# eloialonso/diamond

Measured on NVIDIA H100. Metric: imagined frames/sec (64x64, 3 denoise steps), higher is better.
Workload: dtype fp16 tensor-core operands (split-fp16 on the residual-stream 1x1/conv_in layers), fp32 accumulate, fp32 activations

## Files before the change

diamond_b200/csrc/api.cu:

```cuda
#include <cstdlib>
#include <memory>
#include <mutex>
#include <map>
#include <cuda_runtime.h>

#include <cmath>
#include <cstdarg>
#include <cstdio>
#include <cstring>
#include <functional>
#include <string>
#include <vector>

#include "../../include/diamond_b200.h"
#include "aux_kernels.cuh"
#include "conv_tc.cuh"
#include "wgrad_tc.cuh"
#include "bwd_kernels.cuh"
#include "optim_kernels.cuh"

using namespace dmd;

static thread_local std::string g_err;
static thread_local long long g_launches = 0;
// ... 116 lines not shown
    const int cs[2] = {d->C0, d->C1};
    const int nsrc = d->C1 ? 2 : 1;
    int n = 0;
    for (int rep = 0; rep < (d->precise ? 3 : 1); ++rep)
      for (int k = 0; k < nsrc; ++k) { p->seg_base[n] = (rep == 1) ? lo[k] : hi[k]; p->seg_slabs[n] = cs[k] / 16; ++n; }
    p->Cin = (d->C0 + d->C1) * (d->precise ? 3 : 1);
    p->Cextra = 0;
    if (d->wpk_x) {
      DMD_CHECK(d->xsrc0 && d->xsrc0_lo && d->xC0 > 0 && d->xC0 % 16 == 0 && d->xC1 % 16 == 0 && d->xC0 + d->xC1 <= kMaxCin, "conv: bad fused projection operands");
      DMD_CHECK((d->xC1 == 0) == (d->xsrc1 == nullptr) && (d->xC1 == 0) == (d->xsrc1_lo == nullptr), "conv: fused projection src1 mismatch");
      const uint8_t* xh[2] = {(const uint8_t*)d->xsrc0, (const uint8_t*)d->xsrc1};
      const uint8_t* xl[2] = {(const uint8_t*)d->xsrc0_lo, (const uint8_t*)d->xsrc1_lo};
      const int xc[2] = {d->xC0, d->xC1};
      for (int rep = 0; rep < 2; ++rep)
        for (int k = 0; k < (d->xC1 ? 2 : 1); ++k) {
          DMD_CHECK(n < kMaxSegs, "conv: too many operand segments");
          p->seg_base[n] = (rep == 1) ? xl[k] : xh[k]; p->seg_slabs[n] = xc[k] / 16; ++n;
        }
      p->Cextra = 3 * (d->xC0 + d->xC1);
      p->xslabs = 2 * (d->xC0 + d->xC1) / 16;
      p->wpk_extra = reinterpret_cast<const __half*>(d->wpk_x);
      p->bias_extra = d->bias_x;
    }
    p->nseg = n;
  }
  p->B = d->B; p->H = d->H; p->W = d->W; p->taps = d->taps; p->stride = d->stride;
  if (d->stride == 2) DMD_CHECK(p->H % 2 == 0 && p->W % 2 == 0, "conv: stride 2 needs even H,W");
  p->wpk = reinterpret_cast<const __half*>(d->wpk); p->bias = d->bias; p->Cout = d->Cout; p->CoutPad = d->CoutPad;
  p->resid = d->residual; p->out = d->out; p->ostats = d->out_stats; p->ogs = d->out_gs > 0 ? d->out_gs : d->Cout;
  const Plc g = plc_geometry(d->B, d->H, d->W);
  p->PW = g.PW; p->PH = g.PH; p->Q = g.Q; p->G = g.G; p->plane_bytes = (unsigned long long)g.Qalloc * 16;
  DMD_CHECK((long long)g.Q * (g.PW > g.PH ? g.PW : g.PH) < (1ll << 32), "conv: problem too large for 32-bit position math");
  p->trs = d->wpk_layout == 1 ? 1 : 0;
  if (p->trs) DMD_CHECK(d->taps == 9 && !d->precise && 3 * d->CoutPad <= 256, "conv: row-stacked weights need a 3x3, non-split conv with CoutPad <= 80");
  const int halo = d->taps == 9 ? g.PW + 1 : 0;
  p->P = kTileM + 2 * halo; p->Palloc = p->P | 1;
  if (d->out_stats) {
    const int L4 = d->Cout / 4;
    DMD_CHECK(g.PH * g.PW >= 64, "conv: image too small for the statistics epilogue (a tile may touch at most %d images)", kStatSlots);
    DMD_CHECK(d->Cout % 4 == 0 && (L4 == 4 || L4 == 8 || L4 == 16 || L4 == 32), "conv: out_stats needs Cout in {16,32,64,128} (got %d)", d->Cout);
    DMD_CHECK(d->out_gs == 16 || d->out_gs == 32 || d->out_gs == 64 || d->out_gs == 128, "conv: out_gs must be 16/32/64/128");
    DMD_CHECK(d->Cout % d->out_gs == 0 && d->Cout / d->out_gs <= kMaxOutGroups, "conv: bad output groups");
  }
  p->dPW.init(g.PW); p->dPH.init(g.PH);
  p->num_tiles = (g.Q + kTileM - 1) / kTileM;
  const int kslabs = p->Cin / 16 + p->xslabs;
  const uint32_t w_bytes = conv_weight_bytes(p->taps, p->Cin, p->Cextra, p->CoutPad);
  const ConvSmemLayout L0 = conv_smem_layout(w_bytes, p->Palloc, 0);
  const long long budget = 227ll * 1024 - (long long)L0.total;
  int stages = budget > 0 ? (int)(budget / (long long)L0.slab_bytes) : 0;
  if (stages > 4 * kslabs) stages = 4 * kslabs;
  if (stages > kMaxStages) stages = kMaxStages;
  DMD_CHECK(stages >= 2, "conv: shared memory too small for W=%d Cin=%d CoutPad=%d", p->W, p->Cin, p->CoutPad);
  p->stages = stages;
  *smem = conv_smem_layout(w_bytes, p->Palloc, stages).total;
  *acc_cols = d->CoutPad <= 16 ? 16 : (d->CoutPad <= 32 ? 32 : (d->CoutPad <= 64 ? 64 : 128));
  return 0;
}

struct DevState { int num_sms = 0; void* zeros = nullptr; };
static thread_local int g_num_sms = 0;
static thread_local const uint8_t* g_zeros = nullptr;
static int init_kernels() {
  static std::mutex mu;
  static std::map<int, DevState> states;
  int dev = 0;
  DMD_CUDA(cudaGetDevice(&dev));
  std::lock_guard<std::mutex> lk(mu);
  auto it = states.find(dev);
  if (it == states.end()) {
    DevState st;
    DMD_CUDA(cudaDeviceGetAttribute(&st.num_sms, cudaDevAttrMultiProcessorCount, dev));
    DMD_CUDA(cudaFuncSetAttribute(conv_tc_kernel<16, 9>, cudaFuncAttributeMaxDynamicSharedMemorySize, 227 * 1024));
    DMD_CUDA(cudaFuncSetAttribute(conv_tc_kernel<32, 9>, cudaFuncAttributeMaxDynamicSharedMemorySize, 227 * 1024));
    DMD_CUDA(cudaFuncSetAttribute(conv_tc_kernel<64, 9>, cudaFuncAttributeMaxDynamicSharedMemorySize, 227 * 1024));
    DMD_CUDA(cudaFuncSetAttribute(conv_tc_kernel<128, 9>, cudaFuncAttributeMaxDynamicSharedMemorySize, 227 * 1024));
    DMD_CUDA(cudaFuncSetAttribute(conv_tc_kernel<16, 1>, cudaFuncAttributeMaxDynamicSharedMemorySize, 227 * 1024));
    DMD_CUDA(cudaFuncSetAttribute(conv_tc_kernel<32, 1>, cudaFuncAttributeMaxDynamicSharedMemorySize, 227 * 1024));
    DMD_CUDA(cudaFuncSetAttribute(conv_tc_kernel<64, 1>, cudaFuncAttributeMaxDynamicSharedMemorySize, 227 * 1024));
    DMD_CUDA(cudaFuncSetAttribute(conv_tc_kernel<128, 1>, cudaFuncAttributeMaxDynamicSharedMemorySize, 227 * 1024));
    DMD_CUDA(cudaFuncSetAttribute(wgrad_tc_kernel<16>, cudaFuncAttributeMaxDynamicSharedMemorySize, 227 * 1024));
    DMD_CUDA(cudaFuncSetAttribute(wgrad_tc_kernel<32>, cudaFuncAttributeMaxDynamicSharedMemorySize, 227 * 1024));
    DMD_CUDA(cudaFuncSetAttribute(wgrad_tc_kernel<64>, cudaFuncAttributeMaxDynamicSharedMemorySize, 227 * 1024));
    DMD_CUDA(cudaFuncSetAttribute(attn_cluster_kernel<64>, cudaFuncAttributeMaxDynamicSharedMemorySize, 128 * 1024));
    DMD_CUDA(cudaFuncSetAttribute(attn_cluster_kernel<32>, cudaFuncAttributeMaxDynamicSharedMemorySize, 128 * 1024));
    DMD_CUDA(cudaFuncSetAttribute(attn_kernel<64>, cudaFuncAttributeMaxDynamicSharedMemorySize, 128 * 1024));
    DMD_CUDA(cudaFuncSetAttribute(attn_kernel<32>, cudaFuncAttributeMaxDynamicSharedMemorySize, 128 * 1024));
    DMD_CUDA(cudaFuncSetAttribute(attn_bwd_kernel<64>, cudaFuncAttributeMaxDynamicSharedMemorySize, 200 * 1024));
    DMD_CUDA(cudaFuncSetAttribute(attn_bwd_kernel<32>, cudaFuncAttributeMaxDynamicSharedMemorySize, 200 * 1024));
    DMD_CUDA(cudaFuncSetAttribute(linear_kernel<4>, cudaFuncAttributeMaxDynamicSharedMemorySize, 64 * 1024));
    DMD_CUDA(cudaFuncSetAttribute(linear_kernel<2>, cudaFuncAttributeMaxDynamicSharedMemorySize, 64 * 1024));
    DMD_CUDA(cudaFuncSetAttribute(linear_kernel<1>, cudaFuncAttributeMaxDynamicSharedMemorySize, 64 * 1024));
    DMD_CUDA(cudaMalloc(&st.zeros, 4096));
    DMD_CUDA(cudaMemset(st.zeros, 0, 4096));
    it = states.emplace(dev, st).first;
  }
  g_num_sms = it->second.num_sms;
  g_zeros = (const uint8_t*)it->second.zeros;
  return 0;
}

template <typename Kernel, typename Params>
static int launch_pdl(Kernel kernel, dim3 grid, dim3 block, size_t smem, cudaStream_t st, const Params& p) {
  cudaLaunchConfig_t cfg;
  memset(&cfg, 0, sizeof(cfg));
  cfg.gridDim = grid; cfg.blockDim = block; cfg.dynamicSmemBytes = smem; cfg.stream = st;
  cudaLaunchAttribute attr[1];
  attr[0].id = cudaLaunchAttributeProgrammaticStreamSerialization;
  attr[0].val.programmaticStreamSerializationAllowed = 1;
  cfg.attrs = attr; cfg.numAttrs = tune_int("DMD_NO_PDL", 0) ? 0 : 1;
  DMD_CUDA(cudaLaunchKernelEx(&cfg, kernel, p));
  DMD_LAUNCH_OK();
  return 0;
}

template <int kCols>
static int conv_launch_t(const ConvParams& p0, size_t smem, cudaStream_t st) {
  if (init_kernels()) return 1;
  const int grid = p0.num_tiles < g_num_sms ? p0.num_tiles : g_num_sms;
  ConvParams p = p0;
  p.ktrace = kt_slot(p.taps == 9 ? "conv3x3" : "conv1x1", p.num_tiles, (p.Cin + p.Cextra) * 1000 + p.W);
  if (p.taps == 9) return launch_pdl(conv_tc_kernel<kCols, 9>, dim3(grid), dim3(kConvThreads), smem, st, p);
  return launch_pdl(conv_tc_kernel<kCols, 1>, dim3(grid), dim3(kConvThreads), smem, st, p);
}

static int prep_fill(const dmd_prep_desc* d, PrepParams* p, int* nsrc) {
  DMD_CHECK(d->src0 && d->dst0, "prep: null src0/dst0");
  DMD_CHECK(d->C0 % 8 == 0 && d->C1 % 8 == 0 && d->C0 > 0 && d->C0 <= kMaxCin && d->C1 <= kMaxCin, "prep: channels must be multiples of 8 (C0=%d C1=%d)", d->C0, d->C1);
  DMD_CHECK((d->C1 == 0) == (d->src1 == nullptr) && (d->C1 == 0) == (d->dst1 == nullptr), "prep: src1/dst1/C1 mismatch");
  DMD_CHECK(d->mode >= 0 && d->mode <= 2, "prep: bad mode");
  for (int c : {d->C0, d->C1 ? d->C1 : 16}) {
    const int cp = round_up(c, 16);
    DMD_CHECK(cp == 16 || cp == 32 || cp == 64 || cp == 128, "prep: a source must have <= 16/32/64/128 channels after padding (got %d)", c);
  }
  memset(p, 0, sizeof(*p));
  p->s[0].src = d->src0; p->s[0].C = d->C0; p->s[0].Cpad = round_up(d->C0, 16); p->s[0].stats = d->stats0; p->s[0].gs = d->gs0 > 0 ? d->gs0 : 8;
  p->s[0].c_offset = 0; p->s[0].dst = (uint8_t*)d->dst0; p->s[0].dst_raw = (uint8_t*)d->dst_raw0;
  p->s[0].dst_lo = (uint8_t*)d->dst_lo0; p->s[0].dst_raw_lo = (uint8_t*)d->dst_raw_lo0;
  p->s[1].dst_lo = (uint8_t*)d->dst_lo1; p->s[1].dst_raw_lo = (uint8_t*)d->dst_raw_lo1;
  DMD_CHECK(!(d->dst_raw_lo0 && !d->dst_raw0) && !(d->dst_raw_lo1 && !d->dst_raw1), "prep: raw low part needs the raw operand too");
  p->s[1].src = d->src1; p->s[1].C = d->C1; p->s[1].Cpad = round_up(d->C1 > 0 ? d->C1 : 16, 16); p->s[1].stats = d->stats1; p->s[1].gs = d->gs1 > 0 ? d->gs1 : 8;
  p->s[1].c_offset = d->C0; p->s[1].dst = (uint8_t*)d->dst1; p->s[1].dst_raw = (uint8_t*)d->dst_raw1;
  if (d->mode) {
    DMD_CHECK(d->stats0 && d->gs0 > 0 && d->C0 % d->gs0 == 0, "prep: norm mode needs stats0/gs0");
    if (d->C1) DMD_CHECK(d->stats1 && d->gs1 > 0 && d->C1 % d->gs1 == 0, "prep: norm mode needs stats1/gs1");
    if (d->mode == 1) DMD_CHECK(d->film != nullptr, "prep: AdaGroupNorm needs film");
    if (d->mode == 2) DMD_CHECK(d->gamma && d->beta, "prep: GroupNorm needs gamma/beta");
    DMD_CHECK(d->upsample == 0, "prep: norm + upsample unsupported");
  }
  p->B = d->B; p->Hs = d->Hs; p->Ws = d->Ws; p->ups = d->upsample;
  DMD_CHECK(d->upsample >= 0 && d->upsample <= 2, "prep: upsample must be 0, 1 (nearest 2x) or 2 (zero insertion)");
  DMD_CHECK(d->upsample != 2 || (d->mode == 0 && !d->silu && d->C1 == 0 && !d->dst_raw0 && !d->dst_lo0), "prep: zero insertion is a raw single-source operand");
  p->H = d->upsample ? 2 * d->Hs : d->Hs; p->W = d->upsample ? 2 * d->Ws : d->Ws;
  p->mode = d->mode; p->act = d->silu ? 1 : 0;
  p->film = d->film; p->film_stride = d->film_stride; p->film_off = d->film_off; p->film_ctot = d->C0 + d->C1;
  p->gamma = d->gamma; p->beta = d->beta; p->eps = d->eps;
// ... 2549 lines not shown
```

diamond_b200/csrc/conv_tc.cuh:

```cuda
#pragma once
#include "ptx.cuh"

namespace dmd {

constexpr int kConvThreads = 384;
constexpr int kConvConsumerWarps = 8;
constexpr int kTileM = 128;
constexpr int kMaxCin = 128;
constexpr int kMaxSegs = 8;
constexpr int kMaxStages = 24;
constexpr int kStatSlots = 3;
constexpr int kMaxOutGroups = 4;

struct FastDiv {
  uint32_t d, m;
  __host__ void init(uint32_t dd) {
    d = dd;
    m = (uint32_t)((0x100000000ull / dd) + 1);
  }
  __device__ __forceinline__ uint32_t div(uint32_t n) const { return d == 1 ? n : __umulhi(n, m); }
};

struct Plc {
  int PW, PH, Q, G, Qalloc;
};
__host__ __device__ inline Plc plc_geometry(int B, int H, int W) {
  Plc g;
  g.PW = W + 1; g.PH = H + 1; g.Q = B * g.PH * g.PW; g.G = g.PW + 1;
  g.Qalloc = g.G + ((g.Q + kTileM - 1) / kTileM) * kTileM + kTileM + g.PW + 1;
  return g;
}

struct ConvParams {
  const uint8_t* seg_base[kMaxSegs];
  int seg_slabs[kMaxSegs];
  int nseg;
  int Cin;
  int Cextra;
  const __half* wpk_extra;
  const float* bias_extra;
  int xslabs;
  int B, H, W;
  int taps;
  int stride;
  const __half* wpk;
  const float* bias;
  int Cout, CoutPad;
  const float* resid;
  float* out;
  double* ostats;
  int ogs;
  int PW, PH, Q, G;
  unsigned long long plane_bytes;
  int P, Palloc;
  int num_tiles, stages;
  int trs;
  FastDiv dPW, dPH;
  long long* ktrace;
};

struct ConvSmemLayout {
  uint32_t bias_off, w_off, a_off, slab_bytes, total;
};

__host__ __device__ inline uint32_t conv_weight_bytes(int taps, int Cin, int Cextra, int CoutPad) {
  return (((uint32_t)taps * Cin * CoutPad * 2 + 127u) & ~127u) + (uint32_t)Cextra * CoutPad * 2;
}
__host__ __device__ inline ConvSmemLayout conv_smem_layout(uint32_t w_bytes, int Palloc, int stages) {
  ConvSmemLayout L;
  L.bias_off = 512;
  L.w_off = L.bias_off + 128 * 4;
  L.a_off = (L.w_off + w_bytes + 127u) & ~127u;
  L.slab_bytes = 2u * Palloc * 16;
  L.total = L.a_off + (uint32_t)stages * L.slab_bytes + 16;
  return L;
}

template <int N>
struct RegEpilogue {
  int lane, r0, G;
  float s[kStatSlots][kMaxOutGroups], ss[kStatSlots][kMaxOutGroups];
  int n_cur;

  __device__ __forceinline__ void init(const ConvParams& p, int row0, int lane_) {
    lane = lane_;
    r0 = row0;
    G = p.ostats ? p.Cout / p.ogs : 1;
#pragma unroll
    for (int k = 0; k < kStatSlots; ++k)
#pragma unroll
      for (int g = 0; g < kMaxOutGroups; ++g) s[k][g] = ss[k][g] = 0.f;
    n_cur = -1;
  }

  __device__ __forceinline__ void flush_stats(const ConvParams& p, int img0, int nslots) {
#pragma unroll
    for (int k = 0; k < kStatSlots; ++k) {
#pragma unroll
      for (int g = 0; g < kMaxOutGroups; ++g) {
        if (k < nslots && g < G) {
          float a = s[k][g], b = ss[k][g];
#pragma unroll
          for (int m = 16; m > 0; m >>= 1) {
            a += __shfl_xor_sync(0xffffffffu, a, m);
            b += __shfl_xor_sync(0xffffffffu, b, m);
          }
          if (lane == 0 && img0 + k < p.B && (a != 0.f || b != 0.f)) {
            double* dst = p.ostats + ((size_t)(img0 + k) * G + g) * 2;
            atomicAdd(dst, (double)a);
            atomicAdd(dst + 1, (double)b);
          }
        }
        s[k][g] = ss[k][g] = 0.f;
      }
    }
  }

  template <int kLgs>
  __device__ __forceinline__ void tile(const ConvParams& p, const float* sbias, const float (&acc)[N / 2], int q0) {
    constexpr bool kStats = kLgs > 0;
    constexpr int kGroups = (N / 8) >> kLgs > 0 ? ((N / 8) >> kLgs < kMaxOutGroups ? (N / 8) >> kLgs : kMaxOutGroups) : 1;
    const int n_lo = (int)p.dPH.div(p.dPW.div((uint32_t)q0));
    const int q_last = min(q0 + kTileM, p.Q) - 1;
    const bool single_image = (int)p.dPH.div(p.dPW.div((uint32_t)q_last)) == n_lo;
    if (kStats && n_cur >= 0 && (!single_image || n_lo != n_cur)) { flush_stats(p, n_cur, 1); n_cur = -1; }
    const int c0 = 2 * (lane & 3);
    const bool vec = (p.Cout & 1) == 0;
#pragma unroll
    for (int h = 0; h < 2; ++h) {
      const int q = q0 + r0 + 8 * h;
      int opix = -1, slot = 0;
      if (q < p.Q) {
        const uint32_t R = p.dPW.div((uint32_t)q);
        const int x = q - (int)R * p.PW;
        const int n = (int)p.dPH.div(R);
        const int y = (int)R - n * p.PH;
        bool valid = (x < p.W) && (y < p.H);
        int yo = y, xo = x, Ho = p.H, Wo = p.W;
        if (p.stride == 2) {
          valid = valid && ((x & 1) == 0) && ((y & 1) == 0);
          yo = y >> 1; xo = x >> 1; Ho = p.H >> 1; Wo = p.W >> 1;
        }
        if (valid) { opix = (n * Ho + yo) * Wo + xo; slot = n - n_lo; }
      }
      if (opix < 0) continue;
      float* op = p.out + (size_t)opix * p.Cout;
      const float* rp = p.resid != nullptr ? p.resid + (size_t)opix * p.Cout : nullptr;
      float gs[kMaxOutGroups], gss[kMaxOutGroups];
#pragma unroll
      for (int g = 0; g < kMaxOutGroups; ++g) gs[g] = gss[g] = 0.f;
      constexpr int kBatch = N / 8 < 8 ? N / 8 : 8;
#pragma unroll
      for (int jb = 0; jb < N / 8; jb += kBatch) {
        float2 bv[kBatch], rv[kBatch];
#pragma unroll
        for (int u = 0; u < kBatch; ++u) {
          const int col = 8 * (jb + u) + c0;
          bv[u] = rv[u] = make_float2(0.f, 0.f);
          if (col < p.Cout) {
            bv[u] = make_float2(sbias[col], sbias[col + 1]);
            if (rp) {
              if (vec) rv[u] = __ldg(reinterpret_cast<const float2*>(rp + col));
              else {
                rv[u].x = __ldg(rp + col);
                if (col + 1 < p.Cout) rv[u].y = __ldg(rp + col + 1);
              }
            }
          }
        }
#pragma unroll
        for (int u = 0; u < kBatch; ++u) {
          const int j = jb + u;
          const int col = 8 * j + c0;
          if (col < p.Cout) {
            float2 o = make_float2(acc[4 * j + 2 * h] + bv[u].x, acc[4 * j + 2 * h + 1] + bv[u].y);
            if (vec) {
              if (rp) { o.x += rv[u].x; o.y += rv[u].y; }
              *reinterpret_cast<float2*>(op + col) = o;
            } else {
              if (rp) o.x += rv[u].x;
              op[col] = o.x;
              if (col + 1 < p.Cout) { if (rp) o.y += rv[u].y; op[col + 1] = o.y; } else o.y = 0.f;
            }
            if (kStats) {
              gs[j >> kLgs] += o.x + o.y;
              gss[j >> kLgs] += fmaf(o.x, o.x, o.y * o.y);
            }
          }
        }
      }
      if (kStats) {
        if (single_image) {
#pragma unroll
          for (int g = 0; g < kGroups; ++g) { s[0][g] += gs[g]; ss[0][g] += gss[g]; }
        } else {
#pragma unroll
          for (int k = 0; k < kStatSlots; ++k)
#pragma unroll
            for (int g = 0; g < kGroups; ++g) { s[k][g] += (slot == k) ? gs[g] : 0.f; ss[k][g] += (slot == k) ? gss[g] : 0.f; }
        }
      }
    }
    if (kStats) {
      if (single_image) n_cur = n_lo;
      else { flush_stats(p, n_lo, kStatSlots); n_cur = -1; }
    }
  }

  __device__ __forceinline__ void finish(const ConvParams& p) {
    if (p.ostats != nullptr && n_cur >= 0) flush_stats(p, n_cur, 1);
  }
};

template <int N, int kTaps>
__global__ void __launch_bounds__(kConvThreads, 1) conv_tc_kernel(const ConvParams p) {
  extern __shared__ __align__(128) uint8_t smem[];
  uint64_t* wbar = reinterpret_cast<uint64_t*>(smem);
  uint64_t* full = wbar + 1;
  uint64_t* empty = full + kMaxStages;
  const ConvSmemLayout L = conv_smem_layout(conv_weight_bytes(p.taps, p.Cin, p.Cextra, p.CoutPad), p.Palloc, p.stages);
  float* sbias = reinterpret_cast<float*>(smem + L.bias_off);
  uint8_t* sW = smem + L.w_off;
  uint8_t* sA = smem + L.a_off;

  const int tid = threadIdx.x;
  const int warp = tid >> 5, lane = tid & 31;
  const int halo = (kTaps == 9) ? (p.PW + 1) : 0;
  const int S = p.stages;
  const int main_slabs = p.Cin >> 4;
  const int kslabs = main_slabs + p.xslabs;
  const uint32_t w_main_bytes = ((uint32_t)p.taps * p.Cin * p.CoutPad * 2 + 127u) & ~127u;
  const int tiles_lo = p.num_tiles / (int)gridDim.x, tiles_rem = p.num_tiles % (int)gridDim.x;
  const int tile_begin = (int)blockIdx.x * tiles_lo + min((int)blockIdx.x, tiles_rem);
  const int my_tiles = tiles_lo + ((int)blockIdx.x < tiles_rem ? 1 : 0);

  pdl_launch_dependents();
  if (tid == 0) {
    mbar_init(wbar, 1);
    for (int s = 0; s < S; ++s) { mbar_init(full + s, 1); mbar_init(empty + s, kConvConsumerWarps); }
    fence_mbar_init();
    const uint32_t tap_bytes = (uint32_t)p.Cin * p.CoutPad * 2;
    const uint32_t extra_bytes = (uint32_t)p.Cextra * p.CoutPad * 2;
    mbar_expect_tx(wbar, tap_bytes * p.taps + extra_bytes);
    for (int t = 0; t < p.taps; ++t)
      bulk_g2s(sW + (size_t)t * tap_bytes, reinterpret_cast<const uint8_t*>(p.wpk) + (size_t)t * tap_bytes, tap_bytes, wbar);
    if (extra_bytes) bulk_g2s(sW + w_main_bytes, p.wpk_extra, extra_bytes, wbar);
  }
  for (int i = tid; i < 128; i += blockDim.x)
    sbias[i] = ((p.bias != nullptr && i < p.Cout) ? __ldg(p.bias + i) : 0.f) + ((p.bias_extra != nullptr && i < p.Cout) ? __ldg(p.bias_extra + i) : 0.f);
  __syncthreads();
  pdl_wait();
  if (blockIdx.x == 0 && tid == 128) ktrace_stamp(p.ktrace);

  if (warp < 2) {
    const uint32_t pid = (uint32_t)warp;
    const uint32_t chunk_bytes = (uint32_t)p.P * 16;
    uint32_t stage = 0, phase = 0, nslab = 0;
    for (int it = 0; it < my_tiles; ++it) {
      const size_t pos0 = (size_t)((tile_begin + it) * kTileM - halo + p.G) * 16;
      int seg = 0, seg_ks = 0;
      for (int ks = 0; ks < kslabs; ++ks, ++nslab) {
        if ((nslab & 1u) == pid) {
          mbar_wait(empty + stage, phase ^ 1u);
          if (elect_one_sync()) {
            uint8_t* slab = sA + (size_t)stage * L.slab_bytes;
            const bool xs = ks >= main_slabs;
            const uint32_t bytes = xs ? (uint32_t)kTileM * 16 : chunk_bytes;
            mbar_expect_tx(full + stage, 2 * bytes);
            const uint8_t* plane = p.seg_base[seg] + (size_t)(2 * seg_ks) * p.plane_bytes + pos0 + (xs ? (size_t)halo * 16 : 0);
            bulk_g2s(slab, plane, bytes, full + stage);
            bulk_g2s(slab + (size_t)p.Palloc * 16, plane + p.plane_bytes, bytes, full + stage);
          }
          __syncwarp();
        }
        if (++seg_ks == p.seg_slabs[seg]) { seg_ks = 0; ++seg; }
        if (++stage == (uint32_t)S) { stage = 0; phase ^= 1u; }
      }
    }
  } else if (warp >= 4) {
    const int m0 = ((warp >> 2) - 1) * 64;
    RegEpilogue<N> epi;
    epi.init(p, m0 + 16 * (warp & 3) + (lane >> 2), lane);
    const int lgs = p.ostats ? 31 - __clz(p.ogs >> 3) : 0;
    if (my_tiles > 0) mbar_wait(wbar, 0);
    const uint64_t hi = gmma_desc_hi(128);
    const uint32_t a_lbo = (uint32_t)p.Palloc * 16;
    const uint32_t b_lbo = (uint32_t)(p.trs ? 3 * p.CoutPad : p.CoutPad) * 16;
    const uint32_t x_lbo = (uint32_t)p.CoutPad * 16;
    const uint32_t a_lo0 = (((smem_u32(sA) + (uint32_t)m0 * 16) >> 4) & 0x3FFFu) | (((a_lbo >> 4) & 0x3FFFu) << 16);
    const uint32_t b_lo0 = ((smem_u32(sW) >> 4) & 0x3FFFu) | (((b_lbo >> 4) & 0x3FFFu) << 16);
    const uint32_t b_x0 = (((smem_u32(sW) + w_main_bytes) >> 4) & 0x3FFFu) | (((x_lbo >> 4) & 0x3FFFu) << 16);
    const uint32_t slab16 = L.slab_bytes >> 4;
    const uint32_t kstep16 = (2u * b_lbo) >> 4;
    const uint32_t xstep16 = (2u * x_lbo) >> 4;
    uint32_t shift[kTaps], b_tap[kTaps];
#pragma unroll
    for (int t = 0; t < kTaps; ++t) {
      shift[t] = (uint32_t)(halo + (kTaps == 9 ? (t / 3 - 1) * p.PW + (t % 3 - 1) : 0));
      b_tap[t] = p.trs ? ((uint32_t)(t / 3) * p.Cin * 3u * p.CoutPad * 2 + (uint32_t)(t % 3) * p.CoutPad * 16) >> 4
                       : ((uint32_t)t * p.Cin * p.CoutPad * 2) >> 4;
    }
    const int ng = p.xslabs >> 1;
    float acc[N / 2];
    uint32_t stage = 0, phase = 0, prev = 0;
    int done = 0;
    auto slab = [&](auto issue) {
      mbar_wait(full + stage, phase);
      wgmma_fence();
      issue(a_lo0 + stage * slab16);
      wgmma_commit();
      wgmma_wait<1>();
      if (done > 0 && lane == 0) mbar_arrive(empty + prev);
      prev = stage;
      ++done;
      if (++stage == (uint32_t)S) { stage = 0; phase ^= 1u; }
    };
    for (int it = 0; it < my_tiles; ++it) {
#pragma unroll
      for (int i = 0; i < N / 2; ++i) acc[i] = 0.f;
      done = 0;
      for (int ks = 0; ks < main_slabs; ++ks) {
        const uint32_t b_lo = b_lo0 + (uint32_t)ks * kstep16;
        slab([&](uint32_t a_lo) {
#pragma unroll
          for (int t = 0; t < kTaps; ++t) Wgmma<N>::template mma<0, 0>(acc, hi | (a_lo + shift[t]), hi | (b_lo + b_tap[t]), 1u);
        });
      }
      for (int g = 0; g < ng; ++g)
        slab([&](uint32_t a_lo) {
          Wgmma<N>::template mma<0, 0>(acc, hi | a_lo, hi | (b_x0 + (uint32_t)g * xstep16), 1u);
          Wgmma<N>::template mma<0, 0>(acc, hi | a_lo, hi | (b_x0 + (uint32_t)(2 * ng + g) * xstep16), 1u);
        });
      for (int g = 0; g < ng; ++g)
        slab([&](uint32_t a_lo) { Wgmma<N>::template mma<0, 0>(acc, hi | a_lo, hi | (b_x0 + (uint32_t)(ng + g) * xstep16), 1u); });
      wgmma_wait<0>();
      wgmma_fence_operands(acc);
      if (done > 0 && lane == 0) mbar_arrive(empty + prev);
      const int q0 = (tile_begin + it) * kTileM;
      if (lgs == 0) epi.template tile<0>(p, sbias, acc, q0);
      else if (lgs == 1 || N == 16) epi.template tile<1>(p, sbias, acc, q0);
      else if (lgs == 2 || N == 32) epi.template tile<2>(p, sbias, acc, q0);
      else if (lgs == 3 || N == 64) epi.template tile<3>(p, sbias, acc, q0);
      else epi.template tile<4>(p, sbias, acc, q0);
    }
    epi.finish(p);
  }
}

struct PrepSrc {
  const float* src;
  int C;
  int Cpad;
  const double* stats;
  int gs;
  int c_offset;
  uint8_t* dst;
  uint8_t* dst_lo;
  uint8_t* dst_raw;
  uint8_t* dst_raw_lo;
};
struct PrepParams {
  PrepSrc s[2];
  int B, Hs, Ws, ups, H, W;
  int mode;
  int act;
  const float* film;
  int film_stride, film_off, film_ctot;
  const float* gamma;
  const float* beta;
  float eps;
  int PW, PH, Q, G, Qalloc;
  unsigned long long plane_bytes;
  int pos_per_block;
  FastDiv dPW, dPH;
  long long* ktrace;
};

constexpr int kPrepThreads = 256;
// ... 300 lines not shown
```

diamond_b200/csrc/ptx.cuh:

```cuda
#pragma once
#include <cstdint>
#include <cuda_fp16.h>
#include <cuda_runtime.h>

namespace dmd {

__device__ __forceinline__ uint32_t smem_u32(const void* p) {
  return static_cast<uint32_t>(__cvta_generic_to_shared(p));
}

__device__ __forceinline__ void mbar_init(uint64_t* bar, uint32_t count) {
  asm volatile("mbarrier.init.shared::cta.b64 [%0], %1;" ::"r"(smem_u32(bar)), "r"(count));
}
__device__ __forceinline__ void fence_mbar_init() {
  asm volatile("fence.mbarrier_init.release.cluster;" ::: "memory");
}
__device__ __forceinline__ void mbar_expect_tx(uint64_t* bar, uint32_t bytes) {
  asm volatile("mbarrier.arrive.expect_tx.shared::cta.b64 _, [%0], %1;" ::"r"(smem_u32(bar)), "r"(bytes)
               : "memory");
}
__device__ __forceinline__ void mbar_arrive(uint64_t* bar) {
  asm volatile("mbarrier.arrive.shared::cta.b64 _, [%0];" ::"r"(smem_u32(bar)) : "memory");
}
__device__ __forceinline__ bool mbar_try_wait(uint64_t* bar, uint32_t parity) {
  uint32_t ok;
  asm volatile(
      "{\n\t.reg .pred p;\n\t"
      "mbarrier.try_wait.parity.shared::cta.b64 p, [%1], %2, %3;\n\t"
      "selp.u32 %0, 1, 0, p;\n\t}"
      : "=r"(ok)
      : "r"(smem_u32(bar)), "r"(parity), "r"(1000000u)
      : "memory");
  return ok != 0;
}
__device__ __forceinline__ void mbar_wait(uint64_t* bar, uint32_t parity) {
  uint32_t spins = 0;
  while (!mbar_try_wait(bar, parity)) {
    if (++spins > (1u << 20)) asm volatile("trap;");
  }
}

__device__ __forceinline__ void fence_proxy_async_smem() {
  asm volatile("fence.proxy.async.shared::cta;" ::: "memory");
}

__device__ __forceinline__ void bulk_g2s(void* smem_dst, const void* gsrc, uint32_t bytes, uint64_t* bar) {
  asm volatile(
      "cp.async.bulk.shared::cluster.global.mbarrier::complete_tx::bytes [%0], [%1], %2, [%3];" ::"r"(
          smem_u32(smem_dst)),
      "l"(gsrc), "r"(bytes), "r"(smem_u32(bar))
      : "memory");
}

__host__ __device__ __forceinline__ uint64_t gmma_desc_hi(uint32_t sbo_bytes) {
  return (uint64_t)((sbo_bytes >> 4) & 0x3FFFu) << 32;
}
__device__ __forceinline__ uint64_t gmma_desc(uint32_t saddr, uint32_t lbo_bytes, uint32_t sbo_bytes) {
  return gmma_desc_hi(sbo_bytes) | (uint64_t)((saddr >> 4) & 0x3FFFu) | ((uint64_t)((lbo_bytes >> 4) & 0x3FFFu) << 16);
}

template <int N>
struct Wgmma;
template <>
struct Wgmma<16> {
  template <int kTransA, int kTransB>
  __device__ __forceinline__ static void mma(float (&d)[8], uint64_t adesc, uint64_t bdesc, uint32_t scale_d) {
    asm volatile(
        "{\n\t.reg .pred p;\n\t"
        "setp.ne.b32 p, %10, 0;\n\t"
        "wgmma.mma_async.sync.aligned.m64n16k16.f32.f16.f16 "
        "{%0, %1, %2, %3, %4, %5, %6, %7}, "
        "%8, %9, p, 1, 1, %11, %12;\n\t}"
// ... 30 lines not shown
        : "+f"(d[0]), "+f"(d[1]), "+f"(d[2]), "+f"(d[3]), "+f"(d[4]), "+f"(d[5]), "+f"(d[6]), "+f"(d[7]), "+f"(d[8]), "+f"(d[9]), "+f"(d[10]), "+f"(d[11]), "+f"(d[12]), "+f"(d[13]), "+f"(d[14]), "+f"(d[15]), "+f"(d[16]), "+f"(d[17]), "+f"(d[18]), "+f"(d[19]), "+f"(d[20]), "+f"(d[21]), "+f"(d[22]), "+f"(d[23]), "+f"(d[24]), "+f"(d[25]), "+f"(d[26]), "+f"(d[27]), "+f"(d[28]), "+f"(d[29]), "+f"(d[30]), "+f"(d[31])
        : "l"(adesc), "l"(bdesc), "r"(scale_d), "n"(kTransA), "n"(kTransB)
        : "memory");
  }
};
template <>
struct Wgmma<128> {
  template <int kTransA, int kTransB>
  __device__ __forceinline__ static void mma(float (&d)[64], uint64_t adesc, uint64_t bdesc, uint32_t scale_d) {
    asm volatile(
        "{\n\t.reg .pred p;\n\t"
        "setp.ne.b32 p, %66, 0;\n\t"
        "wgmma.mma_async.sync.aligned.m64n128k16.f32.f16.f16 "
        "{%0, %1, %2, %3, %4, %5, %6, %7, %8, %9, %10, %11, %12, %13, %14, %15, %16, %17, %18, %19, %20, %21, %22, %23, %24, %25, %26, %27, %28, %29, %30, %31, %32, %33, %34, %35, %36, %37, %38, %39, %40, %41, %42, %43, %44, %45, %46, %47, %48, %49, %50, %51, %52, %53, %54, %55, %56, %57, %58, %59, %60, %61, %62, %63}, "
        "%64, %65, p, 1, 1, %67, %68;\n\t}"
        : "+f"(d[0]), "+f"(d[1]), "+f"(d[2]), "+f"(d[3]), "+f"(d[4]), "+f"(d[5]), "+f"(d[6]), "+f"(d[7]), "+f"(d[8]), "+f"(d[9]), "+f"(d[10]), "+f"(d[11]), "+f"(d[12]), "+f"(d[13]), "+f"(d[14]), "+f"(d[15]), "+f"(d[16]), "+f"(d[17]), "+f"(d[18]), "+f"(d[19]), "+f"(d[20]), "+f"(d[21]), "+f"(d[22]), "+f"(d[23]), "+f"(d[24]), "+f"(d[25]), "+f"(d[26]), "+f"(d[27]), "+f"(d[28]), "+f"(d[29]), "+f"(d[30]), "+f"(d[31]), "+f"(d[32]), "+f"(d[33]), "+f"(d[34]), "+f"(d[35]), "+f"(d[36]), "+f"(d[37]), "+f"(d[38]), "+f"(d[39]), "+f"(d[40]), "+f"(d[41]), "+f"(d[42]), "+f"(d[43]), "+f"(d[44]), "+f"(d[45]), "+f"(d[46]), "+f"(d[47]), "+f"(d[48]), "+f"(d[49]), "+f"(d[50]), "+f"(d[51]), "+f"(d[52]), "+f"(d[53]), "+f"(d[54]), "+f"(d[55]), "+f"(d[56]), "+f"(d[57]), "+f"(d[58]), "+f"(d[59]), "+f"(d[60]), "+f"(d[61]), "+f"(d[62]), "+f"(d[63])
        : "l"(adesc), "l"(bdesc), "r"(scale_d), "n"(kTransA), "n"(kTransB)
        : "memory");
  }
};

__device__ __forceinline__ void wgmma_fence() { asm volatile("wgmma.fence.sync.aligned;" ::: "memory"); }
__device__ __forceinline__ void wgmma_commit() { asm volatile("wgmma.commit_group.sync.aligned;" ::: "memory"); }
template <int kPending>
__device__ __forceinline__ void wgmma_wait() {
  asm volatile("wgmma.wait_group.sync.aligned %0;" ::"n"(kPending) : "memory");
}
template <int R>
__device__ __forceinline__ void wgmma_fence_operands(float (&d)[R]) {
#pragma unroll
  for (int i = 0; i < R; ++i) asm volatile("" : "+f"(d[i])::"memory");
}

__device__ __forceinline__ bool elect_one_sync() {
  uint32_t pred;
  asm volatile(
      "{\n"
      ".reg .pred p;\n"
      "elect.sync _|p, 0xffffffff;\n"
      "selp.u32 %0, 1, 0, p;\n"
      "}\n"
      : "=r"(pred));
  return pred != 0;
}

__device__ __forceinline__ void pdl_launch_dependents() { asm volatile("griddepcontrol.launch_dependents;" ::: "memory"); }
__device__ __forceinline__ void pdl_wait() { asm volatile("griddepcontrol.wait;" ::: "memory"); }

__device__ __forceinline__ void ktrace_stamp(long long* slot) {
  if (slot != nullptr) {
    unsigned long long t;
    asm volatile("mov.u64 %0, %%globaltimer;" : "=l"(t));
    *slot = (long long)t;
  }
}

__device__ __forceinline__ float silu_f(float v) {
  float e, r;
  asm("ex2.approx.ftz.f32 %0, %1;" : "=f"(e) : "f"(v * -1.4426950408889634f));
  asm("rcp.approx.ftz.f32 %0, %1;" : "=f"(r) : "f"(1.0f + e));
  return v * r;
}

__device__ __forceinline__ uint32_t pack_h2(float a, float b) {
  __half2 h = __floats2half2_rn(a, b);
  return *reinterpret_cast<uint32_t*>(&h);
// ... 4 lines not shown
```

Measured before the change: 6166.

## Add ping-pong consumer warpgroup pairs to conv kernel with stats handoff

Adds a second pair of consumer warpgroups (kPairs=2) for convs with Cout<=64, so that alternating tiles are processed by different pairs. One pair's epilogue can then overlap the other's WGMMA mainloop, with turn barriers ordering the MMAs and a shared-memory handoff of running GroupNorm statistics between pairs. Register budgets are rebalanced with setmaxnreg. Tile scheduling now skips the trailing padding tiles when no stats are needed, and the per-tap B offsets are computed from new row and column strides instead of precomputed arrays. The change adds barrier complexity and register pressure (112 regs per consumer), and the smaller epilogue batch could slow the epilogue.

```diff
diff --git a/diamond_b200/csrc/api.cu b/diamond_b200/csrc/api.cu
--- a/diamond_b200/csrc/api.cu
+++ b/diamond_b200/csrc/api.cu
@@ -172,6 +172,8 @@
   p->PW = g.PW; p->PH = g.PH; p->Q = g.Q; p->G = g.G; p->plane_bytes = (unsigned long long)g.Qalloc * 16;
   DMD_CHECK((long long)g.Q * (g.PW > g.PH ? g.PW : g.PH) < (1ll << 32), "conv: problem too large for 32-bit position math");
   p->trs = d->wpk_layout == 1 ? 1 : 0;
+  p->b_col16 = p->trs ? (uint32_t)d->CoutPad : ((uint32_t)p->Cin * d->CoutPad * 2) >> 4;
+  p->b_row16 = p->trs ? ((uint32_t)p->Cin * 3u * d->CoutPad * 2) >> 4 : 3u * p->b_col16;
   if (p->trs) DMD_CHECK(d->taps == 9 && !d->precise && 3 * d->CoutPad <= 256, "conv: row-stacked weights need a 3x3, non-split conv with CoutPad <= 80");
   const int halo = d->taps == 9 ? g.PW + 1 : 0;
   p->P = kTileM + 2 * halo; p->Palloc = p->P | 1;
@@ -184,6 +186,7 @@
   }
   p->dPW.init(g.PW); p->dPH.init(g.PH);
   p->num_tiles = (g.Q + kTileM - 1) / kTileM;
+  p->sched_tiles = d->out_stats ? p->num_tiles : (((d->B - 1) * g.PH + d->H - 1) * g.PW + d->W - 1) / kTileM + 1;
   const int kslabs = p->Cin / 16 + p->xslabs;
   const uint32_t w_bytes = conv_weight_bytes(p->taps, p->Cin, p->Cextra, p->CoutPad);
   const ConvSmemLayout L0 = conv_smem_layout(w_bytes, p->Palloc, 0);
@@ -211,14 +214,20 @@
   if (it == states.end()) {
     DevState st;
     DMD_CUDA(cudaDeviceGetAttribute(&st.num_sms, cudaDevAttrMultiProcessorCount, dev));
-    DMD_CUDA(cudaFuncSetAttribute(conv_tc_kernel<16, 9>, cudaFuncAttributeMaxDynamicSharedMemorySize, 227 * 1024));
-    DMD_CUDA(cudaFuncSetAttribute(conv_tc_kernel<32, 9>, cudaFuncAttributeMaxDynamicSharedMemorySize, 227 * 1024));
-    DMD_CUDA(cudaFuncSetAttribute(conv_tc_kernel<64, 9>, cudaFuncAttributeMaxDynamicSharedMemorySize, 227 * 1024));
-    DMD_CUDA(cudaFuncSetAttribute(conv_tc_kernel<128, 9>, cudaFuncAttributeMaxDynamicSharedMemorySize, 227 * 1024));
-    DMD_CUDA(cudaFuncSetAttribute(conv_tc_kernel<16, 1>, cudaFuncAttributeMaxDynamicSharedMemorySize, 227 * 1024));
-    DMD_CUDA(cudaFuncSetAttribute(conv_tc_kernel<32, 1>, cudaFuncAttributeMaxDynamicSharedMemorySize, 227 * 1024));
-    DMD_CUDA(cudaFuncSetAttribute(conv_tc_kernel<64, 1>, cudaFuncAttributeMaxDynamicSharedMemorySize, 227 * 1024));
-    DMD_CUDA(cudaFuncSetAttribute(conv_tc_kernel<128, 1>, cudaFuncAttributeMaxDynamicSharedMemorySize, 227 * 1024));
+    DMD_CUDA(cudaFuncSetAttribute(conv_tc_kernel<16, 9, 1>, cudaFuncAttributeMaxDynamicSharedMemorySize, 227 * 1024));
+    DMD_CUDA(cudaFuncSetAttribute(conv_tc_kernel<32, 9, 1>, cudaFuncAttributeMaxDynamicSharedMemorySize, 227 * 1024));
+    DMD_CUDA(cudaFuncSetAttribute(conv_tc_kernel<64, 9, 1>, cudaFuncAttributeMaxDynamicSharedMemorySize, 227 * 1024));
+    DMD_CUDA(cudaFuncSetAttribute(conv_tc_kernel<128, 9, 1>, cudaFuncAttributeMaxDynamicSharedMemorySize, 227 * 1024));
+    DMD_CUDA(cudaFuncSetAttribute(conv_tc_kernel<16, 1, 1>, cudaFuncAttributeMaxDynamicSharedMemorySize, 227 * 1024));
+    DMD_CUDA(cudaFuncSetAttribute(conv_tc_kernel<32, 1, 1>, cudaFuncAttributeMaxDynamicSharedMemorySize, 227 * 1024));
+    DMD_CUDA(cudaFuncSetAttribute(conv_tc_kernel<64, 1, 1>, cudaFuncAttributeMaxDynamicSharedMemorySize, 227 * 1024));
+    DMD_CUDA(cudaFuncSetAttribute(conv_tc_kernel<128, 1, 1>, cudaFuncAttributeMaxDynamicSharedMemorySize, 227 * 1024));
+    DMD_CUDA(cudaFuncSetAttribute(conv_tc_kernel<16, 9, 2>, cudaFuncAttributeMaxDynamicSharedMemorySize, 227 * 1024));
+    DMD_CUDA(cudaFuncSetAttribute(conv_tc_kernel<32, 9, 2>, cudaFuncAttributeMaxDynamicSharedMemorySize, 227 * 1024));
+    DMD_CUDA(cudaFuncSetAttribute(conv_tc_kernel<64, 9, 2>, cudaFuncAttributeMaxDynamicSharedMemorySize, 227 * 1024));
+    DMD_CUDA(cudaFuncSetAttribute(conv_tc_kernel<16, 1, 2>, cudaFuncAttributeMaxDynamicSharedMemorySize, 227 * 1024));
+    DMD_CUDA(cudaFuncSetAttribute(conv_tc_kernel<32, 1, 2>, cudaFuncAttributeMaxDynamicSharedMemorySize, 227 * 1024));
+    DMD_CUDA(cudaFuncSetAttribute(conv_tc_kernel<64, 1, 2>, cudaFuncAttributeMaxDynamicSharedMemorySize, 227 * 1024));
     DMD_CUDA(cudaFuncSetAttribute(wgrad_tc_kernel<16>, cudaFuncAttributeMaxDynamicSharedMemorySize, 227 * 1024));
     DMD_CUDA(cudaFuncSetAttribute(wgrad_tc_kernel<32>, cudaFuncAttributeMaxDynamicSharedMemorySize, 227 * 1024));
     DMD_CUDA(cudaFuncSetAttribute(wgrad_tc_kernel<64>, cudaFuncAttributeMaxDynamicSharedMemorySize, 227 * 1024));
@@ -257,11 +266,18 @@
 template <int kCols>
 static int conv_launch_t(const ConvParams& p0, size_t smem, cudaStream_t st) {
   if (init_kernels()) return 1;
-  const int grid = p0.num_tiles < g_num_sms ? p0.num_tiles : g_num_sms;
+  const int grid = p0.sched_tiles < g_num_sms ? p0.sched_tiles : g_num_sms;
   ConvParams p = p0;
   p.ktrace = kt_slot(p.taps == 9 ? "conv3x3" : "conv1x1", p.num_tiles, (p.Cin + p.Cextra) * 1000 + p.W);
-  if (p.taps == 9) return launch_pdl(conv_tc_kernel<kCols, 9>, dim3(grid), dim3(kConvThreads), smem, st, p);
-  return launch_pdl(conv_tc_kernel<kCols, 1>, dim3(grid), dim3(kConvThreads), smem, st, p);
+  if constexpr (kCols <= 64) {
+    const size_t smem2 = smem + (p.ostats != nullptr ? kConvHandoffBytes : 0);
+    if (p.sched_tiles > grid && smem2 <= 227 * 1024) {
+      if (p.taps == 9) return launch_pdl(conv_tc_kernel<kCols, 9, 2>, dim3(grid), dim3(conv_threads(2)), smem2, st, p);
+      return launch_pdl(conv_tc_kernel<kCols, 1, 2>, dim3(grid), dim3(conv_threads(2)), smem2, st, p);
+    }
+  }
+  if (p.taps == 9) return launch_pdl(conv_tc_kernel<kCols, 9, 1>, dim3(grid), dim3(conv_threads(1)), smem, st, p);
+  return launch_pdl(conv_tc_kernel<kCols, 1, 1>, dim3(grid), dim3(conv_threads(1)), smem, st, p);
 }
 
 static int prep_fill(const dmd_prep_desc* d, PrepParams* p, int* nsrc) {
diff --git a/diamond_b200/csrc/conv_tc.cuh b/diamond_b200/csrc/conv_tc.cuh
--- a/diamond_b200/csrc/conv_tc.cuh
+++ b/diamond_b200/csrc/conv_tc.cuh
@@ -3,14 +3,18 @@
 
 namespace dmd {
 
-constexpr int kConvThreads = 384;
+__host__ __device__ constexpr int conv_threads(int pairs) { return 128 * (1 + 2 * pairs); }
 constexpr int kConvConsumerWarps = 8;
+constexpr int kProducerRegs2 = 32;
+constexpr int kConsumerRegs2 = 112;
+constexpr int kConvRoles = 256;
 constexpr int kTileM = 128;
 constexpr int kMaxCin = 128;
 constexpr int kMaxSegs = 8;
 constexpr int kMaxStages = 24;
 constexpr int kStatSlots = 3;
 constexpr int kMaxOutGroups = 4;
+constexpr uint32_t kConvHandoffBytes = 2u * kMaxOutGroups * kConvRoles * 4u;
 
 struct FastDiv {
   uint32_t d, m;
@@ -54,6 +58,8 @@
   unsigned long long plane_bytes;
   int P, Palloc;
   int num_tiles, stages;
+  int sched_tiles;
+  uint32_t b_row16, b_col16;
   int trs;
   FastDiv dPW, dPH;
   long long* ktrace;
@@ -76,54 +82,58 @@
   return L;
 }
 
-template <int N>
+template <int N, int kMaxBatch, bool kHandoff>
 struct RegEpilogue {
   int lane, r0, G;
-  float s[kStatSlots][kMaxOutGroups], ss[kStatSlots][kMaxOutGroups];
+  float s[kMaxOutGroups], ss[kMaxOutGroups];
   int n_cur;
-
-  __device__ __forceinline__ void init(const ConvParams& p, int row0, int lane_) {
+  uint32_t xs;
+
+  __device__ __forceinline__ void init(const ConvParams& p, int row0, int lane_, uint32_t xs_) {
     lane = lane_;
     r0 = row0;
     G = p.ostats ? p.Cout / p.ogs : 1;
 #pragma unroll
-    for (int k = 0; k < kStatSlots; ++k)
-#pragma unroll
-      for (int g = 0; g < kMaxOutGroups; ++g) s[k][g] = ss[k][g] = 0.f;
+    for (int g = 0; g < kMaxOutGroups; ++g) s[g] = ss[g] = 0.f;
     n_cur = -1;
-  }
-
-  __device__ __forceinline__ void flush_stats(const ConvParams& p, int img0, int nslots) {
-#pragma unroll
-    for (int k = 0; k < kStatSlots; ++k) {
-#pragma unroll
-      for (int g = 0; g < kMaxOutGroups; ++g) {
-        if (k < nslots && g < G) {
-          float a = s[k][g], b = ss[k][g];
-#pragma unroll
-          for (int m = 16; m > 0; m >>= 1) {
-            a += __shfl_xor_sync(0xffffffffu, a, m);
-            b += __shfl_xor_sync(0xffffffffu, b, m);
-          }
-          if (lane == 0 && img0 + k < p.B && (a != 0.f || b != 0.f)) {
-            double* dst = p.ostats + ((size_t)(img0 + k) * G + g) * 2;
-            atomicAdd(dst, (double)a);
-            atomicAdd(dst + 1, (double)b);
-          }
-        }
-        s[k][g] = ss[k][g] = 0.f;
-      }
-    }
+    xs = xs_;
+  }
+
+  __device__ __forceinline__ void flush_group(const ConvParams& p, int n, int g, float a, float b) const {
+#pragma unroll
+    for (int m = 16; m > 0; m >>= 1) {
+      a += __shfl_xor_sync(0xffffffffu, a, m);
+      b += __shfl_xor_sync(0xffffffffu, b, m);
+    }
+    if (lane == 0 && n < p.B && (a != 0.f || b != 0.f)) {
+      double* dst = p.ostats + ((size_t)n * G + g) * 2;
+      atomicAdd(dst, (double)a);
+      atomicAdd(dst + 1, (double)b);
+    }
+  }
+
+  __device__ __forceinline__ void flush_running(const ConvParams& p) {
+#pragma unroll
+    for (int g = 0; g < kMaxOutGroups; ++g) {
+      if (g < G) flush_group(p, n_cur, g, s[g], ss[g]);
+      s[g] = ss[g] = 0.f;
+    }
+    n_cur = -1;
   }
 
   template <int kLgs>
-  __device__ __forceinline__ void tile(const ConvParams& p, const float* sbias, const float (&acc)[N / 2], int q0) {
+  __device__ __forceinline__ void tile(const ConvParams& p, const float* sbias, const float (&acc)[N / 2], int q0, int it,
+                                       int pair, uint64_t* hand) {
     constexpr bool kStats = kLgs > 0;
     constexpr int kGroups = (N / 8) >> kLgs > 0 ? ((N / 8) >> kLgs < kMaxOutGroups ? (N / 8) >> kLgs : kMaxOutGroups) : 1;
     const int n_lo = (int)p.dPH.div(p.dPW.div((uint32_t)q0));
     const int q_last = min(q0 + kTileM, p.Q) - 1;
     const bool single_image = (int)p.dPH.div(p.dPW.div((uint32_t)q_last)) == n_lo;
-    if (kStats && n_cur >= 0 && (!single_image || n_lo != n_cur)) { flush_stats(p, n_cur, 1); n_cur = -1; }
+    float ms[kStatSlots][kGroups], mss[kStatSlots][kGroups];
+#pragma unroll
+    for (int k = 0; k < kStatSlots; ++k)
+#pragma unroll
+      for (int g = 0; g < kGroups; ++g) ms[k][g] = mss[k][g] = 0.f;
     const int c0 = 2 * (lane & 3);
     const bool vec = (p.Cout & 1) == 0;
 #pragma unroll
@@ -149,7 +159,7 @@
       float gs[kMaxOutGroups], gss[kMaxOutGroups];
 #pragma unroll
       for (int g = 0; g < kMaxOutGroups; ++g) gs[g] = gss[g] = 0.f;
-      constexpr int kBatch = N / 8 < 8 ? N / 8 : 8;
+      constexpr int kBatch = N / 8 < kMaxBatch ? N / 8 : kMaxBatch;
 #pragma unroll
       for (int jb = 0; jb < N / 8; jb += kBatch) {
         float2 bv[kBatch], rv[kBatch];
@@ -192,32 +202,78 @@
       if (kStats) {
         if (single_image) {
 #pragma unroll
-          for (int g = 0; g < kGroups; ++g) { s[0][g] += gs[g]; ss[0][g] += gss[g]; }
+          for (int g = 0; g < kGroups; ++g) { ms[h][g] = gs[g]; mss[h][g] = gss[g]; }
         } else {
 #pragma unroll
           for (int k = 0; k < kStatSlots; ++k)
 #pragma unroll
-            for (int g = 0; g < kGroups; ++g) { s[k][g] += (slot == k) ? gs[g] : 0.f; ss[k][g] += (slot == k) ? gss[g] : 0.f; }
+            for (int g = 0; g < kGroups; ++g) { ms[k][g] += (slot == k) ? gs[g] : 0.f; mss[k][g] += (slot == k) ? gss[g] : 0.f; }
         }
       }
     }
     if (kStats) {
-      if (single_image) n_cur = n_lo;
-      else { flush_stats(p, n_lo, kStatSlots); n_cur = -1; }
-    }
-  }
-
-  __device__ __forceinline__ void finish(const ConvParams& p) {
-    if (p.ostats != nullptr && n_cur >= 0) flush_stats(p, n_cur, 1);
+      if (kHandoff) {
+        n_cur = -1;
+#pragma unroll
+        for (int g = 0; g < kMaxOutGroups; ++g) s[g] = ss[g] = 0.f;
+        if (it > 0) {
+          mbar_wait(hand + pair, (uint32_t)((it - 1) >> 1) & 1u);
+          take_over<kGroups>(p, q0 - kTileM);
+        }
+      }
+      if (n_cur >= 0 && (!single_image || n_lo != n_cur)) flush_running(p);
+      if (single_image) {
+#pragma unroll
+        for (int h = 0; h < 2; ++h)
+#pragma unroll
+          for (int g = 0; g < kGroups; ++g) { s[g] += ms[h][g]; ss[g] += mss[h][g]; }
+        n_cur = n_lo;
+      } else {
+#pragma unroll
+        for (int k = 0; k < kStatSlots; ++k)
+#pragma unroll
+          for (int g = 0; g < kGroups; ++g)
+            if (g < G) flush_group(p, n_lo + k, g, ms[k][g], mss[k][g]);
+      }
+      if (kHandoff) {
+#pragma unroll
+        for (int g = 0; g < kGroups; ++g) { sts_f32(xs + 8 * g * kConvRoles, s[g]); sts_f32(xs + (8 * g + 4) * kConvRoles, ss[g]); }
+        __syncwarp();
+        if (lane == 0) mbar_arrive(hand + (pair ^ 1));
+      }
+    }
+  }
+
+  template <int kGroups>
+  __device__ __forceinline__ void take_over(const ConvParams& p, int q_prev) {
+    const int n_prev = (int)p.dPH.div(p.dPW.div((uint32_t)q_prev));
+    if ((int)p.dPH.div(p.dPW.div((uint32_t)(min(q_prev + kTileM, p.Q) - 1))) == n_prev) n_cur = n_prev;
+#pragma unroll
+    for (int g = 0; g < kGroups; ++g) { s[g] = lds_f32(xs + 8 * g * kConvRoles); ss[g] = lds_f32(xs + (8 * g + 4) * kConvRoles); }
+  }
+
+  __device__ __forceinline__ void finish(const ConvParams& p, bool ran_last, int q_last) {
+    if (p.ostats == nullptr) return;
+    if (kHandoff) {
+      if (!ran_last) return;
+      n_cur = -1;
+#pragma unroll
+      for (int g = 0; g < kMaxOutGroups; ++g) s[g] = ss[g] = 0.f;
+      take_over<kMaxOutGroups>(p, q_last);
+    }
+    if (n_cur >= 0) flush_running(p);
   }
 };
 
-template <int N, int kTaps>
-__global__ void __launch_bounds__(kConvThreads, 1) conv_tc_kernel(const ConvParams p) {
+template <int N, int kTaps, int kPairs>
+__global__ void __launch_bounds__(conv_threads(kPairs), 1) conv_tc_kernel(const ConvParams p) {
+  static_assert(kPairs == 1 || (kPairs == 2 && N <= 64), "two consumer pairs need N <= 64");
   extern __shared__ __align__(128) uint8_t smem[];
   uint64_t* wbar = reinterpret_cast<uint64_t*>(smem);
   uint64_t* full = wbar + 1;
   uint64_t* empty = full + kMaxStages;
+  uint64_t* turn = empty + kMaxStages;
+  uint64_t* hand = turn + 2;
   const ConvSmemLayout L = conv_smem_layout(conv_weight_bytes(p.taps, p.Cin, p.Cextra, p.CoutPad), p.Palloc, p.stages);
   float* sbias = reinterpret_cast<float*>(smem + L.bias_off);
   uint8_t* sW = smem + L.w_off;
@@ -230,14 +286,19 @@
   const int main_slabs = p.Cin >> 4;
   const int kslabs = main_slabs + p.xslabs;
   const uint32_t w_main_bytes = ((uint32_t)p.taps * p.Cin * p.CoutPad * 2 + 127u) & ~127u;
-  const int tiles_lo = p.num_tiles / (int)gridDim.x, tiles_rem = p.num_tiles % (int)gridDim.x;
-  const int tile_begin = (int)blockIdx.x * tiles_lo + min((int)blockIdx.x, tiles_rem);
-  const int my_tiles = tiles_lo + ((int)blockIdx.x < tiles_rem ? 1 : 0);
+  int tile_begin, my_tiles;
+  const auto tile_range = [&]() {
+    const int tiles_lo = p.sched_tiles / (int)gridDim.x, tiles_rem = p.sched_tiles % (int)gridDim.x;
+    tile_begin = (int)blockIdx.x * tiles_lo + min((int)blockIdx.x, tiles_rem);
+    my_tiles = tiles_lo + ((int)blockIdx.x < tiles_rem ? 1 : 0);
+  };
 
   pdl_launch_dependents();
   if (tid == 0) {
     mbar_init(wbar, 1);
     for (int s = 0; s < S; ++s) { mbar_init(full + s, 1); mbar_init(empty + s, kConvConsumerWarps); }
+    if (kPairs == 2)
+      for (int q = 0; q < 2; ++q) { mbar_init(turn + q, kConvConsumerWarps); mbar_init(hand + q, kConvConsumerWarps); }
     fence_mbar_init();
     const uint32_t tap_bytes = (uint32_t)p.Cin * p.CoutPad * 2;
     const uint32_t extra_bytes = (uint32_t)p.Cextra * p.CoutPad * 2;
@@ -252,7 +313,10 @@
   pdl_wait();
   if (blockIdx.x == 0 && tid == 128) ktrace_stamp(p.ktrace);
 
-  if (warp < 2) {
+  if (warp < 4) {
+    if (kPairs == 2) setmaxnreg_dec<kProducerRegs2>();
+    if (warp >= 2) return;
+    tile_range();
     const uint32_t pid = (uint32_t)warp;
     const uint32_t chunk_bytes = (uint32_t)p.P * 16;
     uint32_t stage = 0, phase = 0, nslab = 0;
@@ -277,12 +341,15 @@
         if (++stage == (uint32_t)S) { stage = 0; phase ^= 1u; }
       }
     }
-  } else if (warp >= 4) {
-    const int m0 = ((warp >> 2) - 1) * 64;
-    RegEpilogue<N> epi;
-    epi.init(p, m0 + 16 * (warp & 3) + (lane >> 2), lane);
-    const int lgs = p.ostats ? 31 - __clz(p.ogs >> 3) : 0;
-    if (my_tiles > 0) mbar_wait(wbar, 0);
+  } else {
+    if (kPairs == 2) setmaxnreg_inc<kConsumerRegs2>();
+    tile_range();
+    const int cw = (warp >> 2) - 1;
+    const int pair = cw >> 1;
+    const int m0 = (cw & 1) * 64;
+    RegEpilogue<N, kPairs == 2 ? 4 : 8, kPairs == 2> epi;
+    epi.init(p, m0 + 16 * (warp & 3) + (lane >> 2), lane, smem_u32(smem + L.total) + 4u * ((cw & 1) * 128 + (tid & 127)));
+    if (my_tiles > pair) mbar_wait(wbar, 0);
     const uint64_t hi = gmma_desc_hi(128);
     const uint32_t a_lbo = (uint32_t)p.Palloc * 16;
     const uint32_t b_lbo = (uint32_t)(p.trs ? 3 * p.CoutPad : p.CoutPad) * 16;
@@ -293,57 +360,59 @@
     const uint32_t slab16 = L.slab_bytes >> 4;
     const uint32_t kstep16 = (2u * b_lbo) >> 4;
     const uint32_t xstep16 = (2u * x_lbo) >> 4;
-    uint32_t shift[kTaps], b_tap[kTaps];
-#pragma unroll
-    for (int t = 0; t < kTaps; ++t) {
-      shift[t] = (uint32_t)(halo + (kTaps == 9 ? (t / 3 - 1) * p.PW + (t % 3 - 1) : 0));
-      b_tap[t] = p.trs ? ((uint32_t)(t / 3) * p.Cin * 3u * p.CoutPad * 2 + (uint32_t)(t % 3) * p.CoutPad * 16) >> 4
-                       : ((uint32_t)t * p.Cin * p.CoutPad * 2) >> 4;
-    }
     const int ng = p.xslabs >> 1;
     float acc[N / 2];
-    uint32_t stage = 0, phase = 0, prev = 0;
-    int done = 0;
-    auto slab = [&](auto issue) {
+    uint32_t stage = 0, phase = 0;
+    const auto prev_stage = [&]() { return (stage == 0 ? (uint32_t)S : stage) - 1u; };
+    auto slab = [&](bool release, auto issue) {
       mbar_wait(full + stage, phase);
       wgmma_fence();
       issue(a_lo0 + stage * slab16);
       wgmma_commit();
       wgmma_wait<1>();
-      if (done > 0 && lane == 0) mbar_arrive(empty + prev);
-      prev = stage;
-      ++done;
+      if (release && lane == 0) mbar_arrive(empty + prev_stage());
       if (++stage == (uint32_t)S) { stage = 0; phase ^= 1u; }
     };
-    for (int it = 0; it < my_tiles; ++it) {
+    for (int it = pair; it < my_tiles; it += kPairs) {
+      const uint32_t g0 = (uint32_t)it * (uint32_t)kslabs;
+      stage = g0 % (uint32_t)S;
+      phase = (g0 / (uint32_t)S) & 1u;
+      if (kPairs == 2 && it > 0) mbar_wait(turn + pair, (uint32_t)((it - 1) >> 1) & 1u);
 #pragma unroll
       for (int i = 0; i < N / 2; ++i) acc[i] = 0.f;
-      done = 0;
       for (int ks = 0; ks < main_slabs; ++ks) {
         const uint32_t b_lo = b_lo0 + (uint32_t)ks * kstep16;
-        slab([&](uint32_t a_lo) {
-#pragma unroll
-          for (int t = 0; t < kTaps; ++t) Wgmma<N>::template mma<0, 0>(acc, hi | (a_lo + shift[t]), hi | (b_lo + b_tap[t]), 1u);
+        slab(ks > 0, [&](uint32_t a_lo) {
+          const uint32_t a_c = a_lo + (uint32_t)halo;
+#pragma unroll
+          for (int t = 0; t < kTaps; ++t) {
+            const int dy = kTaps == 9 ? t / 3 : 1, dx = kTaps == 9 ? t % 3 : 1;
+            const uint32_t a_t = a_c + (uint32_t)(dy - 1) * (uint32_t)p.PW + (uint32_t)(dx - 1);
+            const uint32_t b_t = b_lo + (kTaps == 9 ? (uint32_t)dy * p.b_row16 + (uint32_t)dx * p.b_col16 : 0u);
+            Wgmma<N>::template mma<0, 0>(acc, hi | a_t, hi | b_t, 1u);
+          }
         });
       }
       for (int g = 0; g < ng; ++g)
-        slab([&](uint32_t a_lo) {
+        slab(true, [&](uint32_t a_lo) {
           Wgmma<N>::template mma<0, 0>(acc, hi | a_lo, hi | (b_x0 + (uint32_t)g * xstep16), 1u);
           Wgmma<N>::template mma<0, 0>(acc, hi | a_lo, hi | (b_x0 + (uint32_t)(2 * ng + g) * xstep16), 1u);
         });
       for (int g = 0; g < ng; ++g)
-        slab([&](uint32_t a_lo) { Wgmma<N>::template mma<0, 0>(acc, hi | a_lo, hi | (b_x0 + (uint32_t)(ng + g) * xstep16), 1u); });
+        slab(true, [&](uint32_t a_lo) { Wgmma<N>::template mma<0, 0>(acc, hi | a_lo, hi | (b_x0 + (uint32_t)(ng + g) * xstep16), 1u); });
+      if (kPairs == 2 && lane == 0) mbar_arrive(turn + (pair ^ 1));
       wgmma_wait<0>();
       wgmma_fence_operands(acc);
-      if (done > 0 && lane == 0) mbar_arrive(empty + prev);
+      if (lane == 0) mbar_arrive(empty + prev_stage());
       const int q0 = (tile_begin + it) * kTileM;
-      if (lgs == 0) epi.template tile<0>(p, sbias, acc, q0);
-      else if (lgs == 1 || N == 16) epi.template tile<1>(p, sbias, acc, q0);
-      else if (lgs == 2 || N == 32) epi.template tile<2>(p, sbias, acc, q0);
-      else if (lgs == 3 || N == 64) epi.template tile<3>(p, sbias, acc, q0);
-      else epi.template tile<4>(p, sbias, acc, q0);
-    }
-    epi.finish(p);
+      const int lgs = p.ostats ? 31 - __clz(p.ogs >> 3) : 0;
+      if (lgs == 0) epi.template tile<0>(p, sbias, acc, q0, it, pair, hand);
+      else if (lgs == 1 || N == 16) epi.template tile<1>(p, sbias, acc, q0, it, pair, hand);
+      else if (lgs == 2 || N == 32) epi.template tile<2>(p, sbias, acc, q0, it, pair, hand);
+      else if (lgs == 3 || N == 64) epi.template tile<3>(p, sbias, acc, q0, it, pair, hand);
+      else epi.template tile<4>(p, sbias, acc, q0, it, pair, hand);
+    }
+    epi.finish(p, my_tiles > 0 && (my_tiles - 1) % kPairs == pair, (tile_begin + my_tiles - 1) * kTileM);
   }
 }
 
diff --git a/diamond_b200/csrc/ptx.cuh b/diamond_b200/csrc/ptx.cuh
--- a/diamond_b200/csrc/ptx.cuh
+++ b/diamond_b200/csrc/ptx.cuh
@@ -38,6 +38,15 @@
   while (!mbar_try_wait(bar, parity)) {
     if (++spins > (1u << 20)) asm volatile("trap;");
   }
+}
+
+__device__ __forceinline__ float lds_f32(uint32_t addr) {
+  float v;
+  asm volatile("ld.shared.f32 %0, [%1];" : "=f"(v) : "r"(addr) : "memory");
+  return v;
+}
+__device__ __forceinline__ void sts_f32(uint32_t addr, float v) {
+  asm volatile("st.shared.f32 [%0], %1;" ::"r"(addr), "f"(v) : "memory");
 }
 
 __device__ __forceinline__ void fence_proxy_async_smem() {
@@ -134,6 +143,11 @@
   for (int i = 0; i < R; ++i) asm volatile("" : "+f"(d[i])::"memory");
 }
 
+template <int R>
+__device__ __forceinline__ void setmaxnreg_dec() { asm volatile("setmaxnreg.dec.sync.aligned.u32 %0;" ::"n"(R)); }
+template <int R>
+__device__ __forceinline__ void setmaxnreg_inc() { asm volatile("setmaxnreg.inc.sync.aligned.u32 %0;" ::"n"(R)); }
+
 __device__ __forceinline__ bool elect_one_sync() {
   uint32_t pred;
   asm volatile(
```

Result: faster. 6395, median of 6 (+3.7%).
